# usamec/GAML

Hardware: NVIDIA B200
Metric: alignments_scored_per_s (higher is better)
Workload: dtype f64

## Files before the change

gaml_b200/csrc/engine.cu:

```cuda
#include <cuda_runtime.h>
#include <dlfcn.h>

#include <algorithm>
#include <atomic>
#include <climits>
#include <limits>
#include <cmath>
#include <cstdio>
#include <chrono>
#include <cstring>
#include <memory>
#include <memory_resource>
#include <string>
#include <unordered_map>
#include <unordered_set>
#include <vector>

#include "../../include/gaml_b200.h"
#include "kernels.h"
#include "walk_set.h"

namespace gaml {
namespace {

// ... 153 lines not shown
  bool pstar_valid = false;
  DevBuf d_qthr;
  DevBuf d_comb, d_partner12, d_partner21;
  bool comb_ok = false;
  DevBuf d_t2pack;
  bool t2pack_ok = false;
  uint32_t t2base[3] = {0, 0, 0};
  bool pairs_ok = false;
  bool lens_uniform = false;
  uint32_t uniform_ll = 0;
  int32_t class_begin[17] = {0};
  uint32_t cbase[2][5] = {{0}};
  int n_complex = 0;
  bool complex_dirty = true;
  int ins_n = 0;
  double floor_a = 0, floor_b = 0;
  DevBuf d_state_acc;
  bool total_valid = false;
  int total_two_len = 0;
  bool has_state = false;
  FlatCache flat_cache;
  int bad_bases = 0;
  bool penalty = false;
  bool sharded = false;
  bool penalty_pending = false;
  std::vector<unsigned long long> h_type1;
  DevBuf d_cov_thr, d_ev, d_ev_sorted, d_ev_temp, d_bad;
  bool pb_penalty = false;
  DevBuf d_pb_ikey, d_pb_iend, d_pb_pkey, d_pb_packed, d_pb_runmax, d_pb_temp, d_pb_count;
  std::vector<int4> h_pb_seeds, h_pb_occ;
  std::vector<uint32_t> h_pb_prefix;
  std::vector<int> h_pb_walk_len;
  std::vector<int> h_bad;
  cudaEvent_t ev0 = nullptr, ev1 = nullptr;
  ~ReadSetState() {
    for (cudaEvent_t e : {ev0, ev1})
      if (e) cudaEventDestroy(e);
  }
};

struct SetPlan {
  bool full = true;
  bool delta_only = false;
  int n_erased = 0;
  int total_len = 0;
  int64_t records = 0;
  int64_t touch_records = 0;
  int64_t records1 = 0;
  int n_cov_walks = 0, n_type1 = 0;
  uint32_t ev_cap = 0;
  size_t type1_off = 0, csbegin_off = 0, cs_off = 0, evcount_off = 0;
  int grid = 0;
  int cgrid = 0;
  size_t occ_off[2] = {0, 0};
  size_t touch_off = 0, prefix_off = 0;
  size_t pstar_off = 0;
  int n_touch = 0;
  size_t pb_seeds_off = 0, pb_occ_off = 0, pb_prefix_off = 0, pb_len_off = 0;
  uint32_t pb_cap = 0;
  size_t mtouch_off = 0, mprefix_off = 0;
  int n_mtouch = 0, n_mtouch1 = 0;
  int64_t multi_records = 0;
};

}
}
// ... 42 lines not shown
  DevBuf d_flags, d_scratch, d_csr_temp, d_logtab;
  DevBuf d_batch_blob, d_batch_acc, d_batch_out;
  DevBuf d_aln[8];
  std::vector<double> h_batch_out;
  void* h_append_pinned = nullptr;
  size_t h_append_cap = 0;
  cudaEvent_t ev_append = nullptr;
  bool append_copy_pending = false;
  double* h_out = nullptr;
  double* d_out_mapped = nullptr;
  std::vector<double> h_res;
  double* exch_host = nullptr;
  double* exch_dev = nullptr;
  int exch_rank = 0, exch_world = 1;
  bool exch_owned = false;
  DevBuf d_peer_lines, d_peer_table;
  std::vector<void*> peer_ptrs;
  std::vector<char> peer_opened;
  int peer_rank = 0, peer_world = 0;
  bool peer_on = false;
  unsigned long long* h_gather = nullptr;
  unsigned long long* d_gather_mapped = nullptr;
  void* nccl_lib = nullptr;
  void* nccl_comm = nullptr;
  int nccl_rank = 0, nccl_world = 0;
  bool nccl_on = false;
  DevBuf d_part, d_part_sum;
  unsigned long long exchange_timeout_ns = 20ull * 1000 * 1000 * 1000;
  struct GraphEntry { cudaGraph_t graph = nullptr; cudaGraphExec_t exec = nullptr; std::vector<cudaGraphNode_t> nodes; };
  std::unordered_map<uint64_t, GraphEntry> graphs;
  bool use_graphs = true;
  bool running_total = true;
  bool timing_pending = false;
  size_t h_out_cap = 0;
  unsigned long long scratch_entries = 1ull << 22;
  uint32_t ovf_cap = 1u << 20;
  uint32_t epoch = 0;
  uint32_t stamp_gen = 0;
  bool capacity_grew = false;
  bool prepared = false, launched = false;
  std::vector<SetPlan> plan;
  WalkSet wsets[2];
  int cur_set = 0;
  WalkSet& cur() { return wsets[cur_set]; }
  WalkSet& prev() { return wsets[cur_set ^ 1]; }
  std::vector<SlotUpdate> h_updates;
  std::vector<std::vector<Occ>> h_occs;
  std::vector<std::vector<TouchRange>> h_touches, h_mtouches;
  std::vector<OccBuilder> h_ob;
  std::vector<WalkView> h_refs;
  std::vector<Walk> h_walks;
  bool fast_changes = true;
  bool permute_reads = true;
  bool append_enabled = true;
  HashCounts prev_counts;
  bool have_prev = false;
  WalkDiff cur_diff;
  int prev_total_len = 0, cur_total_len = 0;
  Changes h_changes;
  alignas(16) char pool_buf[1 << 18];
  std::pmr::monotonic_buffer_resource pool{pool_buf, sizeof(pool_buf)};
  int n_updates = 0;
  size_t upd_off = 0, blob_bytes = 0;
  gaml_stats stats{};
};

// ... 1609 lines not shown
  CU(cudaGetLastError());
  return GAML_OK;
}

int nccl_all_reduce_doubles(gaml_ctx* ctx, double* buf, size_t count) {
  NcclApi* api = nccl_api(&ctx->error);
  if (!api || !ctx->nccl_comm) return fail(ctx, GAML_ERR_STATE, "no NCCL communicator: gaml_nccl_exchange_init first");
  const int rc = api->all_reduce(buf, buf, count,  8,  0, ctx->nccl_comm, ctx->stream);
  if (rc != 0) return fail(ctx, GAML_ERR_CUDA, std::string("ncclAllReduce: ") + (api->get_error_string ? api->get_error_string(rc) : "error"));
  return GAML_OK;
}

int ensure_gather_area(gaml_ctx* ctx, int world) {
  if (ctx->h_gather) return GAML_OK;
  (void)world;
  const size_t words = ((size_t)64 * GAML_EXCHANGE_MAX_SETS + 1) * kResultStride;
  CU(cudaHostAlloc(reinterpret_cast<void**>(&ctx->h_gather), words * 8, cudaHostAllocMapped));
  memset(ctx->h_gather, 0, words * 8);
  CU(cudaHostGetDevicePointer(reinterpret_cast<void**>(&ctx->d_gather_mapped), ctx->h_gather, 0));
  return GAML_OK;
}

int launch(gaml_ctx* ctx) {
  if (!ctx->prepared) return fail(ctx, GAML_ERR_STATE, "gaml_eval_launch without gaml_eval_prepare");
  cudaStream_t st = ctx->stream;
  const size_t n_sets = ctx->sets.size();
  if (ctx->timeline) {
    CU(ctx->d_timeline.reserve(kTimelineWords * 8, 0, true, st));
    CU(cudaMemsetAsync(ctx->d_timeline.p, 0, kTimelineWords * 8, st));
  }
  char* blob = ctx->blob_dev;
  int launches = 0;
  bool any_penalty = false;
  for (auto& rs : ctx->sets) any_penalty |= rs->penalty || rs->pb_penalty;
  LaunchList chain;
  const bool record = ctx->use_graphs && !ctx->profile && !any_penalty && ctx->sets.size() <= 3;
  struct RecorderGuard { ~RecorderGuard() { set_launch_recorder(nullptr); } } recorder_guard;
  if (record) set_launch_recorder(&chain);
  else if (ctx->timed) CU(cudaEventRecord(ctx->ev[0], st));
  launch_apply_slots(reinterpret_cast<const SlotUpdate*>(blob + ctx->upd_off), ctx->n_updates,
                     reinterpret_cast<const SlotUpdate*>(blob + ctx->patch_upd_off), ctx->n_patch,
                     reinterpret_cast<const int32_t*>(blob + ctx->patch_skip_off), ctx->n_skip, ctx->d_tables.as<SlotA*>(),
                     ctx->d_tables.as<SlotB*>() + ctx->stores.size(), ctx->d_tables.as<SlotA*>() + 2 * ctx->stores.size(),
                     ctx->d_tables.as<const int32_t*>() + 3 * ctx->stores.size(),
                     ctx->stores.size() <= (size_t)kInlineStores ? &ctx->h_tables : nullptr, ctx->epoch, ctx->d_flags.as<unsigned long long>(),
                     (int)flags_words(n_sets), ctx->timeline ? ctx->d_timeline.as<unsigned long long>() : nullptr, st);
  launches++;
  int64_t records = 0, reads = 0, bytes = 0;
  bool any_full = false;
  const bool profile = ctx->profile;
  bool chained = true;
  for (size_t s = 0; s < n_sets; s++) {
    ReadSetState& rs = *ctx->sets[s];
    const SetPlan& sp = ctx->plan[s];
    ScoreParams P = make_params(ctx, s);
    const int og = overflow_grid(ctx->sm_count);
    records += sp.records;
    reads += rs.n_local;
    if (rs.penalty) {
      CU(rs.d_ev.reserve((size_t)sp.ev_cap * 8, 0, false, st));
      CU(rs.d_ev_sorted.reserve((size_t)sp.ev_cap * 8, 0, false, st));
      CU(rs.d_ev_temp.reserve(std::max<size_t>(coverage_sort_temp_bytes(sp.ev_cap), 256), 0, false, st));
      CU(rs.d_bad.reserve(std::max<size_t>(sp.n_cov_walks, 1) * 4, 0, false, st));
      P.ev_keys = rs.d_ev.as<unsigned long long>();
      CU(cudaMemsetAsync(rs.d_ev.p, 0xff, (size_t)sp.ev_cap * 8, st));
      CU(cudaMemsetAsync(rs.d_bad.p, 0, std::max<size_t>(sp.n_cov_walks, 1) * 4, st));
      if (sp.n_type1) CU(cudaMemcpyAsync(rs.d_ev.p, blob + sp.type1_off, (size_t)sp.n_type1 * 8, cudaMemcpyDeviceToDevice, st));
      CU(cudaMemcpyAsync(P.ev_count, blob + sp.evcount_off, 4, cudaMemcpyDeviceToDevice, st));
      chained = false;
    }
    if (rs.cfg.kind == GAML_KIND_PAIRED) {
      if (sp.full) {
        const uint32_t n_multi = (uint32_t)sp.multi_records;
        launches += launch_paired_full(P, sp.grid, sp.cgrid, n_multi, og, ctx->sm_count, st, chained, profile, rs.ev0, rs.ev1);
        any_full = true;
        bytes += 16 * sp.records + 12 * (int64_t)rs.n_local;
      } else {
        launch_paired_delta(P, (uint32_t)sp.touch_records, sp.grid, og, ctx->sm_count, st, chained, profile, rs.ev0, rs.ev1);
        launches += sp.delta_only ? (sp.touch_records > 0 ? 2 : 1) : (sp.touch_records > 0 ? 3 : 1);
        bytes += 16 * sp.records + (sp.delta_only ? 0 : 12 * (int64_t)rs.n_local);
      }
      if (rs.penalty && rs.sharded) {
        chained = false;
      } else if (rs.penalty) {
        CU(launch_coverage(rs.d_ev.as<unsigned long long>(), rs.d_ev_sorted.as<unsigned long long>(), sp.ev_cap, rs.d_ev_temp.p,
                           rs.d_ev_temp.cap, reinterpret_cast<const int*>(blob + sp.csbegin_off),
                           reinterpret_cast<const int*>(blob + sp.cs_off), rs.cfg.step,
                           rs.cfg.insert_mean + 5 * rs.cfg.insert_std, rs.d_bad.as<int>(), ctx->sm_count, st));
        launches += 3;
        chained = false;
      } else {
        chained = !(profile && !sp.full);
      }
    } else if (rs.cfg.kind == GAML_KIND_SINGLE) {
      launch_single_full(P, sp.grid, sp.cgrid, og, st, chained, profile, rs.ev0, rs.ev1);
      chained = true;
      launches += 2 + (sp.cgrid > 0);
      bytes += 16 * sp.records + 12 * (int64_t)rs.n_local;
    } else {
      launch_pacbio_full(P, sp.grid, og, st, chained, profile, rs.ev0, rs.ev1);
      chained = true;
      launches += 2;
      if (rs.pb_penalty) {
        const size_t cap = sp.pb_cap;
        CU(rs.d_pb_ikey.reserve(cap * 2 * 8, 0, false, st));
        CU(rs.d_pb_iend.reserve(cap * 2 * 4, 0, false, st));
        CU(rs.d_pb_pkey.reserve(cap * 4 * 8, 0, false, st));
// ... 29 lines not shown
    }
  }
  if (ctx->peer_on && n_sets > 0) {
    const unsigned long long* gen = ctx->d_peer_lines.as<unsigned long long>() +
                                    (size_t)(ctx->epoch & 1u) * (size_t)ctx->peer_world * GAML_EXCHANGE_MAX_SETS * kResultStride;
    launch_exchange_gather(gen, ctx->peer_world, (int)n_sets, GAML_EXCHANGE_MAX_SETS, ctx->epoch, ctx->d_gather_mapped,
                           ctx->d_gather_mapped + (size_t)ctx->peer_world * GAML_EXCHANGE_MAX_SETS * kResultStride,
                           ctx->exchange_timeout_ns, st);
    launches++;
  }
  if (record) {
    set_launch_recorder(nullptr);
    const int rc = replay_chain(ctx, chain);
    if (rc != GAML_OK) return rc;
  }
  if (!record && ctx->timed) CU(cudaEventRecord(ctx->ev[3], st));
  if (nccl_lines(ctx) && n_sets > 0) {
    const int rc = nccl_reduce_lines(ctx, (int)n_sets);
    if (rc != GAML_OK) return rc;
    launches++;
  }
  CU(cudaGetLastError());
  ctx->stats.kernel_launches += launches;
  ctx->stats.last_records_gathered = records;
  ctx->stats.last_reads_scanned = reads;
  ctx->stats.last_algorithmic_bytes = bytes;
  ctx->stats.last_was_full = any_full ? 1 : 0;
  for (size_t s = 0; s < n_sets; s++)
    if (ctx->plan[s].delta_only) ctx->stats.delta_only_evals++;
  ctx->launched = true;
  return GAML_OK;
}

int wait_line(gaml_ctx* ctx, const volatile uint64_t* line, uint64_t want_bits, double* dst, bool own) {
  unsigned spins = 0;
  const auto t0 = std::chrono::steady_clock::now();
  for (;;) {
    uint64_t w[8];
    for (int j = 0; j < 8; j++) w[j] = line[j];
    uint64_t sum = kResultSeal;
    for (int j = 0; j < 7; j++) sum ^= w[j];
    if (w[6] == want_bits && w[7] == sum) {
      memcpy(dst, w, sizeof(w));
      return GAML_OK;
    }
    cpu_relax();
    if ((++spins & 0x3fffu) == 0) {
      const cudaError_t q = cudaStreamQuery(ctx->stream);
      if (q != cudaSuccess && q != cudaErrorNotReady) {
        ctx->error = std::string("evaluation failed on the device: ") + cudaGetErrorString(q);
        return GAML_ERR_CUDA;
      }
      const double waited = std::chrono::duration<double>(std::chrono::steady_clock::now() - t0).count();
      if (own && q == cudaSuccess && waited > 1.0) return fail(ctx, GAML_ERR_CUDA, "evaluation finished without publishing its result");
      if (!own && waited > 60.0) return fail(ctx, GAML_ERR_STATE, "a peer rank did not publish its result within 60 s");
    }
  }
}

int finish(gaml_ctx* ctx, double* partials, int32_t* total_len, double* gathered = nullptr) {
  if (!ctx->launched) return fail(ctx, GAML_ERR_STATE, "gaml_eval_finish without gaml_eval_launch");
  const size_t n_sets = ctx->sets.size();
  if (gathered && !ctx->exch_host && !ctx->peer_on && !ctx->nccl_on)
    return fail(ctx, GAML_ERR_STATE, "gaml_eval_finish_gathered needs a result exchange (gaml_set_result_exchange, gaml_peer_exchange_open "
                                     "or gaml_nccl_exchange_init)");
  const double want_d = (double)ctx->epoch;
  uint64_t want_bits;
  memcpy(&want_bits, &want_d, 8);
  const int gather_world = ctx->peer_on ? ctx->peer_world : (ctx->nccl_on ? ctx->nccl_world : ctx->exch_world);
  const bool peer_gather = gathered && ctx->peer_on;
  if (peer_gather) {
    const size_t flag_at = (size_t)ctx->peer_world * GAML_EXCHANGE_MAX_SETS * kResultStride;
    double flag[kResultStride];
    const int rc = wait_line(ctx, reinterpret_cast<const volatile uint64_t*>(ctx->h_gather + flag_at), want_bits, flag, true);
    if (rc != GAML_OK) return rc;
    std::atomic_thread_fence(std::memory_order_acquire);
// ... 5 lines not shown
      return fail(ctx, GAML_ERR_STATE, "a peer rank did not publish its result in time (ranks out of lockstep?)");
    }
  }
  const double* own_lines = peer_gather ? reinterpret_cast<const double*>(ctx->h_gather) + (size_t)ctx->peer_rank * n_sets * kResultStride
                            : (ctx->exch_host ? ctx->exch_host + exch_line(ctx, ctx->exch_rank, 0) * kResultStride : ctx->h_out);
  bool need_sync = false;
  for (size_t s = 0; s < n_sets; s++) {
    ReadSetState& rs = *ctx->sets[s];
    if ((rs.pb_penalty || rs.penalty) && rs.sharded) {
      rs.penalty_pending = true;
      need_sync = true;
      continue;
    }
    if (rs.pb_penalty) {
      rs.h_bad.assign(1, 0);
      CU(cudaMemcpyAsync(rs.h_bad.data(), rs.d_bad.p, 4, cudaMemcpyDeviceToHost, ctx->stream));
      need_sync = true;
      continue;
    }
    if (!rs.penalty) continue;
    rs.h_bad.assign(std::max(ctx->plan[s].n_cov_walks, 1), 0);
    if (ctx->plan[s].n_cov_walks)
      CU(cudaMemcpyAsync(rs.h_bad.data(), rs.d_bad.p, (size_t)ctx->plan[s].n_cov_walks * 4, cudaMemcpyDeviceToHost, ctx->stream));
    need_sync = true;
  }
  ctx->h_res.resize(std::max<size_t>(n_sets, 1) * kResultStride);
  if (need_sync) {
    CU(cudaStreamSynchronize(ctx->stream));
    memcpy(ctx->h_res.data(), own_lines, n_sets * kResultStride * sizeof(double));
  } else if (peer_gather) {
    memcpy(ctx->h_res.data(), own_lines, n_sets * kResultStride * sizeof(double));
  } else {
    const volatile uint64_t* ho = reinterpret_cast<const volatile uint64_t*>(own_lines);
    for (size_t s = 0; s < n_sets; s++) {
      const int rc = wait_line(ctx, ho + s * kResultStride, want_bits, ctx->h_res.data() + s * kResultStride, true);
      if (rc != GAML_OK) return rc;
    }
    std::atomic_thread_fence(std::memory_order_acquire);
  }
  if (gathered) {
    for (int rk = 0; rk < gather_world; rk++)
      for (size_t s = 0; s < n_sets; s++) {
        double line[kResultStride];
        if (nccl_lines(ctx)) {
          if (rk == 0) {
            const int rc = wait_line(ctx, reinterpret_cast<const volatile uint64_t*>(ctx->h_gather + s * kResultStride), want_bits, line, true);
            if (rc != GAML_OK) return rc;
            if (((uint64_t)line[5]) & 15) {
              for (auto& rsp : ctx->sets) rsp->has_state = rsp->total_valid = false;
            }
          } else {
            memset(line, 0, sizeof(line));
          }
        } else if (peer_gather) {
          memcpy(line, reinterpret_cast<const double*>(ctx->h_gather) + ((size_t)rk * n_sets + s) * kResultStride, sizeof(line));
          if (rk != ctx->peer_rank && (((uint64_t)line[5]) & 15)) return fail(ctx, GAML_ERR_CAPACITY, "a peer rank reported a capacity error");
        } else if (rk == ctx->exch_rank) {
          memcpy(line, ctx->h_res.data() + s * kResultStride, sizeof(line));
        } else {
          const volatile uint64_t* src = reinterpret_cast<const volatile uint64_t*>(ctx->exch_host + exch_line(ctx, rk, s) * kResultStride);
          const int rc = wait_line(ctx, src, want_bits, line, false);
          if (rc != GAML_OK) return rc;
          if (((uint64_t)line[5]) & 15) return fail(ctx, GAML_ERR_CAPACITY, "a peer rank reported a capacity error");
        }
        for (int k = 0; k < GAML_PARTIAL_DOUBLES; k++) gathered[((size_t)rk * n_sets + s) * GAML_PARTIAL_DOUBLES + k] = line[k];
      }
  }
  ctx->stats.last_d2h_bytes = (int64_t)(n_sets * kResultStride * sizeof(double));
  ctx->timing_pending = ctx->timed;
  if (!ctx->timed) ctx->stats.last_device_ms = ctx->stats.last_score_kernel_ms = 0;
  ctx->stats.evals++;
  ctx->prepared = ctx->launched = false;
  int tl = 0;
  uint32_t flags = 0, ovf = 0;
  int64_t scratch_placements = 0;
  bool any_paired = false;
  for (size_t s = 0; s < n_sets; s++) {
    ReadSetState& rs = *ctx->sets[s];
    const double* o = ctx->h_res.data() + s * kResultStride;
    if (partials)
      for (int k = 0; k < GAML_PARTIAL_DOUBLES; k++) partials[s * GAML_PARTIAL_DOUBLES + k] = o[k];
    const uint64_t f = (uint64_t)o[5];
    flags |= (uint32_t)(f & 15);
    ovf += (uint32_t)((f >> 4) & 0xffffff);
    scratch_placements = std::max<int64_t>(scratch_placements, (int64_t)(f >> 28));
    if (rs.pb_penalty && !rs.sharded) rs.bad_bases = rs.h_bad[0];
    if (rs.cfg.kind == GAML_KIND_PAIRED) {
      if (rs.penalty && !rs.sharded) {
        if (ctx->plan[s].full) rs.bad_bases = 0;
        for (int w = 0; w < ctx->plan[s].n_cov_walks; w++)
          rs.bad_bases += w < ctx->plan[s].n_erased ? -rs.h_bad[w] : rs.h_bad[w];
      }
      {
        const int tl1 = ctx->plan[s].total_len == 0 ? 1 : ctx->plan[s].total_len;
        rs.total_two_len = (int)(2u * (unsigned)tl1);
        rs.total_valid = true;
      }
      rs.has_state = true;
      any_paired = true;
    }
  }
  if (any_paired) {
    const WalkSet& now = ctx->cur();
    const WalkDiff& d = ctx->cur_diff;
    if (ctx->have_prev && d.valid && ctx->prev_counts.valid && !ctx->prev_counts.crowded()) {
      const WalkSet& was = ctx->prev();
      for (int i : d.old_changed) ctx->prev_counts.add(was.hash[i], -1);
      for (int i : d.new_changed) ctx->prev_counts.add(now.hash[i], +1);
    } else {
      ctx->prev_counts.rebuild(now);
    }
    ctx->prev_total_len = ctx->cur_total_len;
    ctx->cur_set ^= 1;
    ctx->have_prev = true;
    ctx->cur_diff.valid = false;
  }
  for (int kind = 0; kind < 3; kind++)
    for (size_t s = 0; s < n_sets; s++)
      if (ctx->sets[s]->cfg.kind == kind) tl = ctx->plan[s].total_len;
  if (total_len) *total_len = tl;
// ... 1435 lines not shown
}

int gaml_set_profiling(gaml_ctx* ctx, int32_t level) {
  if (check_ctx(ctx)) return GAML_ERR_ARG;
  ctx->timed = level == 1 || level == 2;
  ctx->profile = level == 2;
  ctx->timeline = level == 3;
  return GAML_OK;
}

int gaml_read_timeline(gaml_ctx* ctx, double* out_us, int32_t n) {
  if (check_ctx(ctx) || !out_us || n < kTimelineWords) return GAML_ERR_ARG;
  if (!ctx->timeline || !ctx->d_timeline.p) return fail(ctx, GAML_ERR_STATE, "gaml_set_profiling(ctx, 3) and one evaluation first");
  cudaSetDevice(ctx->device);
  CU(cudaMemcpyAsync(ctx->h_timeline, ctx->d_timeline.p, kTimelineWords * 8, cudaMemcpyDeviceToHost, ctx->stream));
  CU(cudaStreamSynchronize(ctx->stream));
  unsigned long long t0 = ~0ull;
  for (int k = 0; k < kTimelineWords; k += 2)
    if (ctx->h_timeline[k]) t0 = std::min(t0, ~ctx->h_timeline[k]);
  for (int k = 0; k < kTimelineWords; k += 2) {
    const bool ran = ctx->h_timeline[k] != 0;
    out_us[k] = ran ? (double)(~ctx->h_timeline[k] - t0) * 1e-3 : -1.0;
    out_us[k + 1] = ran ? (double)(ctx->h_timeline[k + 1] - t0) * 1e-3 : -1.0;
  }
  return GAML_OK;
}

int gaml_get_stats(gaml_ctx* ctx, gaml_stats* out) {
  if (check_ctx(ctx) || !out) return GAML_ERR_ARG;
  if (ctx->timing_pending) {
    cudaSetDevice(ctx->device);
    float ms = 0, ms2 = 0;
    if (cudaEventSynchronize(ctx->ev[3]) == cudaSuccess) cudaEventElapsedTime(&ms, ctx->ev[0], ctx->ev[3]);
    if (ctx->profile)
      for (auto& rs : ctx->sets) {
        float t = 0;
        if (cudaEventElapsedTime(&t, rs->ev0, rs->ev1) == cudaSuccess) ms2 += t;
      }
    ctx->stats.last_device_ms = ms;
    ctx->stats.last_score_kernel_ms = ms2;
    ctx->timing_pending = false;
  }
  ctx->stats.cache_appends = ctx->stats.cache_rebuilds = 0;
  for (auto& rs : ctx->sets) {
    ctx->stats.cache_appends += rs->appends;
    ctx->stats.cache_rebuilds += rs->rebuilds;
  }
  *out = ctx->stats;
  return GAML_OK;
}

}
```

gaml_b200/csrc/kernels.cu:

```cuda
#include <cub/device/device_radix_sort.cuh>
#include <cub/device/device_scan.cuh>

#include <chrono>
#include <cstdio>
#include <cstdlib>
#include <cstring>
#include <type_traits>
#include <utility>

#include "kernels.h"

namespace gaml {

namespace {

constexpr int kCapLong = 8;
constexpr int kBlock = 256;
constexpr int kOvfBlock = 128;

__device__ __forceinline__ int4 ldg4(const void* p) { return __ldg(reinterpret_cast<const int4*>(p)); }
__device__ __forceinline__ uint4 ldg_stream(const uint4* p) {
  uint4 v;
  asm volatile("ld.global.nc.L1::no_allocate.v4.u32 {%0,%1,%2,%3}, [%4];" : "=r"(v.x), "=r"(v.y), "=r"(v.z), "=r"(v.w) : "l"(p));
  return v;
// ... 72 lines not shown
  __syncthreads();
  if (threadIdx.x == 0) {
    unsigned __int128 x = 0;
#pragma unroll
    for (int j = 0; j < 8; j++) x += (unsigned __int128)sm[j] << (16 * j);
#pragma unroll
    for (int j = 0; j < 4; j++) {
      const unsigned long long limb = (unsigned long long)(unsigned)(x >> (32 * j));
      if (limb) atomicAdd(accum + j, limb);
    }
    if (sm[8]) atomicAdd(accum + 4, (unsigned long long)(long long)(int)sm[8]);
    if (sm[9]) atomicAdd(accum + 5, (unsigned long long)(long long)(int)sm[9]);
    if (sm[10]) atomicAdd(accum + 6, (unsigned long long)(long long)(int)sm[10]);
  }
}

struct PublishArgs {
  const unsigned long long* accum;
  unsigned long long* state_acc;
  double* out;
  const uint32_t* error_flag;
  const uint32_t* ovf_count;
  const unsigned long long* scratch_cursor;
  uint32_t* ticket;
  uint32_t* done;
  uint32_t epoch;
  int32_t state_add;
  long long ql;
  long long n_reads;
  unsigned long long* const* peer_bufs;
  int32_t peer_world;
  uint32_t peer_line;
  double* part_out;
};
__device__ __forceinline__ PublishArgs publish_args(const ScoreParams& P, uint32_t* ticket) {
  return PublishArgs{P.accum, P.state_acc, P.out, P.error_flag, P.ovf_count, P.scratch_cursor, ticket, P.done, P.epoch, P.state_add,
                     P.ql, (long long)P.n_reads, P.peer_bufs, P.peer_world, P.peer_line, P.part_out};
}

__device__ __noinline__ void publish_set(PublishArgs A) {
  const int lane = threadIdx.x & 31;
  unsigned long long w[8] = {0, 0, 0, 0, 0, 0, 0, 0};
  if (lane == 0) {
    __threadfence();
    unsigned long long a[7];
    for (int j = 0; j < 7; j++) a[j] = __ldcg(A.accum + j);
    unsigned __int128 x = 0;
    for (int j = 0; j < 4; j++) x += (unsigned __int128)a[j] << (32 * j);
    if (A.state_acc) {
      if (A.state_add) {
        x += ((unsigned __int128)__ldcg(A.state_acc + 1) << 64) | (unsigned __int128)__ldcg(A.state_acc);
        for (int j = 4; j < 7; j++) a[j] += __ldcg(A.state_acc + j - 2);
      }
      A.state_acc[0] = (unsigned long long)x;
      A.state_acc[1] = (unsigned long long)(x >> 64);
      for (int j = 4; j < 7; j++) A.state_acc[j - 2] = a[j];
    }
    const long long n_log = A.n_reads - (long long)a[4] - (long long)a[5] - (long long)a[6];
    const __int128 v = (__int128)x - (__int128)n_log * (__int128)A.ql;
    const unsigned __int128 xv = (unsigned __int128)v;
    const unsigned long long scratch = __ldcg(A.scratch_cursor);
    w[0] = (unsigned long long)__double_as_longlong((double)(long long)(v >> 40));
    w[1] = (unsigned long long)__double_as_longlong((double)(unsigned long long)(xv & (((unsigned __int128)1 << 40) - 1)));
    w[2] = (unsigned long long)__double_as_longlong((double)a[4]);
    w[3] = (unsigned long long)__double_as_longlong((double)a[5]);
    w[4] = (unsigned long long)__double_as_longlong((double)a[6]);
    w[5] = (unsigned long long)__double_as_longlong((double)__ldcg(A.error_flag) + 16.0 * (double)min(__ldcg(A.ovf_count), 0xffffffu) +
                                                    268435456.0 * (double)min(scratch, 0xffffffull));
    w[6] = (unsigned long long)__double_as_longlong((double)A.epoch);
    w[7] = kResultSeal;
    for (int j = 0; j < 7; j++) w[7] ^= w[j];
  }
  unsigned long long mine = 0;
#pragma unroll
  for (int j = 0; j < 8; j++) {
    const unsigned long long v = __shfl_sync(0xffffffffu, w[j], 0);
    if (lane == j) mine = v;
  }
  if (lane < 8) reinterpret_cast<unsigned long long*>(A.out)[lane] = mine;
  if (A.part_out && lane < 8) reinterpret_cast<unsigned long long*>(A.part_out)[lane] = mine;
  if (A.peer_bufs) {
    for (int p = 0; p < A.peer_world; p++) {
      unsigned long long* dst = A.peer_bufs[p] + (size_t)A.peer_line * kResultStride;
      if (lane < 8) dst[lane] = mine;
    }
    __threadfence_system();
  }
}

__global__ void __launch_bounds__(kResultStride * 32) exchange_gather_kernel(const unsigned long long* lines, int world, int n_sets, int max_sets,
                                                                              uint32_t epoch, unsigned long long* host_lines,
                                                                              unsigned long long* host_flag, unsigned long long timeout_ns) {
  pdl_release();
  __shared__ int s_fail;
  if (threadIdx.x == 0) s_fail = 0;
  __syncthreads();
  const unsigned long long want = (unsigned long long)__double_as_longlong((double)epoch);
  const unsigned long long t0 = global_ns();
  for (int i = threadIdx.x; i < world * n_sets; i += blockDim.x) {
    const int rk = i / n_sets, st = i % n_sets;
    const volatile unsigned long long* src = lines + ((size_t)rk * max_sets + st) * kResultStride;
    unsigned long long w[8];
// ... 5 lines not shown
      for (int j = 0; j < 7; j++) sum ^= w[j];
      if (w[6] == want && w[7] == sum) break;
      if (global_ns() - t0 > timeout_ns) {
        s_fail = 1;
        break;
      }
    }
    unsigned long long* dst = host_lines + (size_t)i * kResultStride;
#pragma unroll
    for (int j = 0; j < 8; j++) dst[j] = w[j];
  }
  __threadfence_system();
  __syncthreads();
  if (threadIdx.x < 8) {
    unsigned long long w[8] = {(unsigned long long)s_fail, 0, 0, 0, 0, 0, want, kResultSeal};
    for (int j = 0; j < 7; j++) w[7] ^= w[j];
    host_flag[threadIdx.x] = w[threadIdx.x];
  }
}

__global__ void reduced_publish_kernel(const double* reduced, int n_sets, uint32_t epoch, unsigned long long* host_lines) {
  const int s = blockIdx.x * blockDim.x + threadIdx.x;
  if (s >= n_sets) return;
  unsigned long long w[8];
  for (int j = 0; j < 6; j++) w[j] = (unsigned long long)__double_as_longlong(reduced[(size_t)s * kResultStride + j]);
  w[6] = (unsigned long long)__double_as_longlong((double)epoch);
  w[7] = kResultSeal;
  for (int j = 0; j < 7; j++) w[7] ^= w[j];
  __threadfence_system();
  for (int j = 0; j < 8; j++) host_lines[(size_t)s * kResultStride + j] = w[j];
}

__device__ __noinline__ void finish_blocks(PublishArgs A, bool early) {
  __shared__ bool s_last;
  __threadfence();
  __syncthreads();
  if (threadIdx.x == 0) {
    bool last = atomicAdd(A.ticket, 1u) == gridDim.x - 1;
    if (last && early) {
      __threadfence();
      last = __ldcg(A.ovf_count) == 0;
    }
    s_last = last;
  }
  __syncthreads();
  if (!s_last || threadIdx.x >= 32) return;
  publish_set(A);
  if (early && threadIdx.x == 0) *A.done = 1u;
}
__device__ __forceinline__ void finish_set(const ScoreParams& P) { finish_blocks(publish_args(P, P.ticket2), false); }
__device__ __forceinline__ void finish_set_if_complete(const ScoreParams& P) { finish_blocks(publish_args(P, P.ticket), true); }

__device__ __noinline__ double slow_log(double v) { return log(v); }

__device__ __forceinline__ double table_log(const double2* __restrict__ tab, double v) {
  const long long ix = __double_as_longlong(v);
  if ((unsigned long long)(ix - 0x0010000000000000ll) >= 0x7fe0000000000000ull) return slow_log(v);
  const long long tmp = ix - 0x3fe6000000000000ll;
  const int i = (int)((tmp >> 45) & 127);
  const long long k = tmp >> 52;
  const double z = __longlong_as_double(ix - (tmp & 0xfff0000000000000ll));
  const double2 e = tab[i];
  const double r = fma(z, e.x, -1.0);
  double p = fma(r, 1.0 / 7.0, -1.0 / 6.0);
  p = fma(r, p, 0.2);
  p = fma(r, p, -0.25);
  p = fma(r, p, 1.0 / 3.0);
  p = fma(r, p, -0.5);
  p = fma(r * r, p, r);
  return fma((double)k, 0.693147180559945309417232121458, e.y) + p;
}

__device__ __forceinline__ void acc_term(Acc& a, unsigned& floored, const double2* log_tab, double p, double pstar, long long qthr) {
  if (p < pstar) {
    floored++;
    acc_add_q(a, qthr);
    return;
  }
  const double lg = table_log(log_tab, p);
  if (fabs(lg) < kFixLimit) acc_add_q(a, __double2ll_rn(lg * kFixScale));
  else acc_count_odd(a, lg);
// ... 2334 lines not shown
  static_assert(sizeof...(KArgs) <= sizeof(PendingLaunch::arg_ptrs) / sizeof(void*), "too many kernel arguments");
  static_assert((sizeof(KArgs) + ... + 0) + 16 * sizeof...(KArgs) <= sizeof(PendingLaunch::arg_buf), "argument buffer too small");
  PendingLaunch local;
  LaunchList* rec = g_recorder;
  PendingLaunch& pl = (rec && rec->n < 16) ? rec->item[rec->n] : local;
  pl.func = reinterpret_cast<const void*>(kernel);
  pl.grid = (unsigned)grid;
  pl.block = (unsigned)block;
  pl.pdl = pdl;
  pl.n_args = 0;
  size_t off = 0;
  (pack_arg<std::remove_cv_t<std::remove_reference_t<KArgs>>>(pl, off, static_cast<std::remove_cv_t<std::remove_reference_t<KArgs>>>(args)), ...);
  if (rec && rec->n < 16) {
    rec->n++;
    return;
  }
  issue_launch(pl, st);
}

void launch_apply_slots(const SlotUpdate* upd, int n, const SlotUpdate* patch, int n_patch, const int32_t* skip, int n_skip,
                        SlotA* const* tab_a, SlotB* const* tab_b, SlotA* const* comb_base,
                        const int32_t* const* comb_map, const StoreTables* inline_tabs, uint32_t epoch, unsigned long long* flags,
                        int n_flag_words, unsigned long long* timeline, cudaStream_t st) {
  const int m = n + n_patch > n_flag_words ? n + n_patch : n_flag_words;
  if (inline_tabs)
    launch_chain(apply_slots_kernel<true>, (m + 255) / 256, 256, st, false, upd, n, patch, n_patch, skip, n_skip, tab_a, tab_b, comb_base,
                 comb_map, *inline_tabs, epoch, flags, n_flag_words, timeline);
  else
    launch_chain(apply_slots_kernel<false>, (m + 255) / 256, 256, st, false, upd, n, patch, n_patch, skip, n_skip, tab_a, tab_b, comb_base,
                 comb_map, StoreTables{}, epoch, flags, n_flag_words, timeline);
}

int launch_paired_full(const ScoreParams& P, int grid, int cgrid, uint32_t n_multi_items, int ovf_grid, int sm_count,
                       cudaStream_t st, bool chained, bool profile, cudaEvent_t e0, cudaEvent_t e1) {
  int n_launched = 0;
  (void)cgrid;
  ScoreParams Q = P;
  bool dep = chained && !profile;
  bool first = true;
  if (n_multi_items > 0 || P.n_appx > 0) {
    Q.chain_first = 1;
    Q.finish_here = 0;
    if (n_multi_items < (uint32_t)P.n_appx) n_multi_items = (uint32_t)P.n_appx;
    static const int per_sm = resident_blocks(paired_multi_kernel, kOvfBlock);
    launch_chain(paired_multi_kernel, grid_for(n_multi_items, kOvfBlock, sm_count, per_sm), kOvfBlock, st, dep, Q);
    n_launched++;
    dep = true;
    first = false;
  }
  if (profile) cudaEventRecord(e0, st);
  Q.chain_first = first || profile ? 1 : 0;
  Q.finish_here = profile ? 0 : 1;
  {
    static StreamKernel seen[16];
    static int seen_per_sm[16];
    static int n_seen = 0;
    auto blocks_per_sm = [&](StreamKernel k) {
      for (int i = 0; i < n_seen; i++)
        if (seen[i] == k) return seen_per_sm[i];
      const int v = resident_blocks(k, kBlock);
      if (n_seen < 16) { seen[n_seen] = k; seen_per_sm[n_seen++] = v; }
      return v;
    };
    const bool tab = P.pairs != nullptr && P.comb != nullptr && P.fast != nullptr;
    const StreamKernel k = stream_kernel(P.ev_keys != nullptr, P.pairs != nullptr, tab);
    if (k) {
      grid = grid_for((size_t)P.n_reads, kBlock, sm_count, blocks_per_sm(k));
      launch_chain(k, grid, kBlock, st, dep && !profile, Q);
      n_launched++;
    } else {
      ScoreParams Q1 = Q;
      Q1.finish_here = 0;
      const StreamKernel k1 = stream_kernel_tier1(), k2 = stream_kernel_rest();
      launch_chain(k1, grid_for((size_t)std::max(P.n_tier1, 1), kBlock, sm_count, blocks_per_sm(k1)), kBlock, st, dep && !profile, Q1);
      ScoreParams Q2 = Q;
      Q2.chain_first = 0;
      const int items = std::max(std::max(P.n_main, P.n_complex - P.n_main), std::max(P.n_cross / 2, P.n_appx));
      launch_chain(k2, grid_for((size_t)std::max(items, 1), kBlock, sm_count, blocks_per_sm(k2)), kBlock, st, true, Q2);
      n_launched += 2;
    }
  }
  if (profile) cudaEventRecord(e1, st);
  launch_chain(paired_overflow_kernel, ovf_grid, kOvfBlock, st, !profile, P, 1);
  return n_launched + 1;
}

void launch_paired_delta(const ScoreParams& P, uint32_t n_touch_records, int grid_total, int ovf_grid, int sm_count,
                         cudaStream_t st, bool chained, bool profile, cudaEvent_t e0, cudaEvent_t e1) {
  if (profile) cudaEventRecord(e0, st);
  bool dep = chained && !profile;
  if (n_touch_records > 0) {
    static const int per_sm = resident_blocks(paired_delta_kernel, kOvfBlock);
    launch_chain(paired_delta_kernel, grid_for(n_touch_records, kOvfBlock, sm_count, per_sm), kOvfBlock, st, dep, P);
    dep = true;
  }
  if (P.delta_only) {
    launch_chain(paired_overflow_kernel, n_touch_records > 0 ? ovf_grid : 1, kOvfBlock, st, dep, P, 2);
  } else {
    if (n_touch_records > 0) launch_chain(paired_overflow_kernel, ovf_grid, kOvfBlock, st, true, P, 0);
    launch_chain(paired_total_kernel, grid_total, kBlock, st, dep, P);
  }
  if (profile) cudaEventRecord(e1, st);
}

void launch_single_full(const ScoreParams& P, int grid, int cgrid, int ovf_grid, cudaStream_t st, bool chained, bool profile,
                        cudaEvent_t e0, cudaEvent_t e1) {
  if (profile) cudaEventRecord(e0, st);
  launch_chain(single_full_kernel, grid, kBlock, st, chained && !profile, P);
  if (cgrid > 0) launch_chain(single_complex_kernel, cgrid, kBlock, st, true, P);
  if (profile) cudaEventRecord(e1, st);
  launch_chain(single_overflow_kernel, ovf_grid, kOvfBlock, st, !profile, P);
}

void launch_pacbio_full(const ScoreParams& P, int grid, int ovf_grid, cudaStream_t st, bool chained, bool profile, cudaEvent_t e0,
                        cudaEvent_t e1) {
  if (profile) cudaEventRecord(e0, st);
  launch_chain(pacbio_full_kernel, grid, kBlock, st, chained && !profile, P);
// ... 400 lines not shown
```

gaml_b200/csrc/kernels.h:

```cpp
#pragma once
#include <cuda_runtime.h>

#include "device_types.h"

namespace gaml {

struct PendingLaunch {
  const void* func = nullptr;
  unsigned grid = 1, block = 1;
  bool pdl = false;
  int n_args = 0;
  void* arg_ptrs[16];
  alignas(16) unsigned char arg_buf[1536];
};
struct LaunchList {
  PendingLaunch item[16];
  int n = 0;
};
void set_launch_recorder(LaunchList* list);
cudaError_t issue_launch(const PendingLaunch& pl, cudaStream_t st);

enum { kGridPairedFull = 0, kGridPairedComplex, kGridPairedTotal, kGridSingleFull, kGridSingleComplex, kGridPacbioFull };
int score_grid(int which, int n_items, int sm_count);
int overflow_grid(int sm_count);

constexpr int kInlineStores = 8;
struct StoreTables {
  SlotA* a[kInlineStores];
  SlotB* b[kInlineStores];
  SlotA* cb[kInlineStores];
  const int32_t* cm[kInlineStores];
};
void launch_apply_slots(const SlotUpdate* upd, int n, const SlotUpdate* patch, int n_patch, const int32_t* skip, int n_skip,
                        SlotA* const* tab_a, SlotB* const* tab_b, SlotA* const* comb_base,
                        const int32_t* const* comb_map, const StoreTables* inline_tabs, uint32_t epoch, unsigned long long* flags,
                        int n_flag_words, unsigned long long* timeline, cudaStream_t st);
constexpr int kTimelineWords = 12;
int launch_paired_full(const ScoreParams& P, int grid, int cgrid, uint32_t n_multi_items, int ovf_grid, int sm_count,
                       cudaStream_t st, bool chained, bool profile, cudaEvent_t e0, cudaEvent_t e1);
void launch_paired_delta(const ScoreParams& P, uint32_t n_touch_records, int grid_total, int ovf_grid, int sm_count, cudaStream_t st,
                         bool chained, bool profile, cudaEvent_t e0, cudaEvent_t e1);
void launch_single_full(const ScoreParams& P, int grid, int cgrid, int ovf_grid, cudaStream_t st, bool chained, bool profile,
                        cudaEvent_t e0, cudaEvent_t e1);
void launch_pacbio_full(const ScoreParams& P, int grid, int ovf_grid, cudaStream_t st, bool chained, bool profile, cudaEvent_t e0,
                        cudaEvent_t e1);

cudaError_t build_csr(const void* arena, size_t n_records, int n_reads, bool is_long, uint32_t* rowptr, uint32_t* cursor,
                      void* rows, void* first, void* temp, size_t temp_bytes, int sm_count, cudaStream_t st, int* launches);
cudaError_t build_complex_list(const void* first1, const void* first2, int n_reads, uint32_t* flags, uint32_t* list,
                               void* temp, size_t temp_bytes, cudaStream_t st, int* launches, uint32_t* n_complex_out,
                               int32_t* class_begin);
void launch_pack_tier2(const void* cdesc, const void* rows1, const void* rows2, const int32_t* class_begin, const uint32_t cbase[2][5],
                       const uint32_t tbase[3], void* out, uint32_t* bad, cudaStream_t st);
void launch_pack_pairs(const void* first1, const void* first2, int n, const int32_t* partner12, void* out, uint32_t* bad, cudaStream_t st);
void launch_cdesc_fill(const uint32_t* list, int n_complex, const uint32_t* lens, const uint32_t* cptr1, const uint32_t* cptr2,
                       void* desc, cudaStream_t st);
cudaError_t compact_offsets(const uint32_t* list, int n_complex, const uint32_t* rowptr, uint32_t* cptr, const uint32_t* lens,
                            uint32_t* clens, void* temp, size_t temp_bytes, cudaStream_t st, int* launches);
cudaError_t compact_copy(const uint32_t* list, int n_complex, const uint32_t* rowptr, const uint32_t* cptr, const void* rows,
                         void* crows, cudaStream_t st, int* launches);
void launch_batch(const ScoreParams& P, const BatchParams& B, uint32_t n_touch_records, double* out, const uint32_t* error_flag,
                  int sm_count, cudaStream_t st);
int batch_hist_bins(int n_len);
int batch_launches(int n_len, bool touch);
void launch_build_term_table(const double* p1, const double* p2, const double* ins, int ins_n, int shift, const void* log_tab, void* out,
                             int sm_count, cudaStream_t st);
cudaError_t build_fast_pairs(const void* pairs, int n, int shift, int ins_n, uint32_t uniform_ll, void* fast, uint32_t* flags, uint32_t* list,
                             void* temp, size_t temp_bytes, cudaStream_t st, int* launches);
struct AppendGroupHost { uint32_t read, new_begin, n_new, dst; };
struct AppendMate {
  const void* arena_src; void* arena_dst; uint32_t n_rec;
  const void* groups; int n_groups; const void* new_rows; void* rows; void* first;
// ... 30 lines not shown
```

Measured before the change: 137.5 billion.

## Launch paired overflow tail kernel on demand instead of every full evaluation

When graphs are recorded and no peer/NCCL exchange is active, the paired full path now omits the overflow kernel from the chain. The main kernel publishes a 'pending' result (negative epoch) if overflow entries exist, and the host then launches the tail kernel and waits again. A per-set keep_tail flag, set from the previous overflow count, keeps the tail in the chain when overflow was seen last time. This removes an always-present launch from the common path, but adds a host round trip when overflow does occur, and the extra tail time is added to the reported timing.

```diff
diff --git a/gaml_b200/csrc/engine.cu b/gaml_b200/csrc/engine.cu
--- a/gaml_b200/csrc/engine.cu
+++ b/gaml_b200/csrc/engine.cu
@@ -209,6 +209,10 @@
   std::vector<uint32_t> h_pb_prefix;
   std::vector<int> h_pb_walk_len;
   std::vector<int> h_bad;
+  bool keep_tail = false;
+  bool tail_on_demand = false;
+  ScoreParams tail_params{};
+  int tail_grid = 0;
   cudaEvent_t ev0 = nullptr, ev1 = nullptr;
   ~ReadSetState() {
     for (cudaEvent_t e : {ev0, ev1})
@@ -317,6 +321,7 @@
   bool use_graphs = true;
   bool running_total = true;
   bool timing_pending = false;
+  bool tail_timed = false;
   size_t h_out_cap = 0;
   unsigned long long scratch_entries = 1ull << 22;
   uint32_t ovf_cap = 1u << 20;
@@ -1992,7 +1997,11 @@
   char* blob = ctx->blob_dev;
   int launches = 0;
   bool any_penalty = false;
-  for (auto& rs : ctx->sets) any_penalty |= rs->penalty || rs->pb_penalty;
+  for (auto& rs : ctx->sets) {
+    any_penalty |= rs->penalty || rs->pb_penalty;
+    rs->tail_on_demand = false;
+  }
+  ctx->tail_timed = false;
   LaunchList chain;
   const bool record = ctx->use_graphs && !ctx->profile && !any_penalty && ctx->sets.size() <= 3;
   struct RecorderGuard { ~RecorderGuard() { set_launch_recorder(nullptr); } } recorder_guard;
@@ -2032,7 +2041,13 @@
     if (rs.cfg.kind == GAML_KIND_PAIRED) {
       if (sp.full) {
         const uint32_t n_multi = (uint32_t)sp.multi_records;
-        launches += launch_paired_full(P, sp.grid, sp.cgrid, n_multi, og, ctx->sm_count, st, chained, profile, rs.ev0, rs.ev1);
+        rs.tail_on_demand = record && !ctx->peer_on && !nccl_lines(ctx) && !rs.keep_tail;
+        if (rs.tail_on_demand) {
+          rs.tail_params = P;
+          rs.tail_grid = og;
+        }
+        launches += launch_paired_full(P, sp.grid, sp.cgrid, n_multi, og, ctx->sm_count, st, chained, profile, rs.ev0, rs.ev1,
+                                       !rs.tail_on_demand);
         any_full = true;
         bytes += 16 * sp.records + 12 * (int64_t)rs.n_local;
       } else {
@@ -2128,7 +2143,8 @@
   return GAML_OK;
 }
 
-int wait_line(gaml_ctx* ctx, const volatile uint64_t* line, uint64_t want_bits, double* dst, bool own) {
+int wait_line(gaml_ctx* ctx, const volatile uint64_t* line, uint64_t want_bits, double* dst, bool own, bool* pending = nullptr,
+              uint64_t pend_bits = 0) {
   unsigned spins = 0;
   const auto t0 = std::chrono::steady_clock::now();
   for (;;) {
@@ -2136,8 +2152,10 @@
     for (int j = 0; j < 8; j++) w[j] = line[j];
     uint64_t sum = kResultSeal;
     for (int j = 0; j < 7; j++) sum ^= w[j];
-    if (w[6] == want_bits && w[7] == sum) {
+    const bool alt = pending && w[6] == pend_bits;
+    if ((w[6] == want_bits || alt) && w[7] == sum) {
       memcpy(dst, w, sizeof(w));
+      if (pending) *pending = alt;
       return GAML_OK;
     }
     cpu_relax();
@@ -2209,9 +2227,35 @@
     memcpy(ctx->h_res.data(), own_lines, n_sets * kResultStride * sizeof(double));
   } else {
     const volatile uint64_t* ho = reinterpret_cast<const volatile uint64_t*>(own_lines);
+    const double pend_d = -(double)ctx->epoch;
+    uint64_t pend_bits;
+    memcpy(&pend_bits, &pend_d, 8);
+    bool any_pending = false;
     for (size_t s = 0; s < n_sets; s++) {
-      const int rc = wait_line(ctx, ho + s * kResultStride, want_bits, ctx->h_res.data() + s * kResultStride, true);
+      ReadSetState& rs = *ctx->sets[s];
+      bool pending = false;
+      const int rc = wait_line(ctx, ho + s * kResultStride, want_bits, ctx->h_res.data() + s * kResultStride, true,
+                               rs.tail_on_demand ? &pending : nullptr, pend_bits);
       if (rc != GAML_OK) return rc;
+      if (!pending) continue;
+      if (!any_pending && ctx->timed) CU(cudaEventRecord(ctx->ev[1], ctx->stream));
+      any_pending = true;
+      launch_paired_tail(rs.tail_params, rs.tail_grid, ctx->stream);
+      CU(cudaGetLastError());
+      ctx->stats.kernel_launches++;
+    }
+    if (any_pending) {
+      if (ctx->timed) {
+        CU(cudaEventRecord(ctx->ev[2], ctx->stream));
+        ctx->tail_timed = true;
+      }
+      for (size_t s = 0; s < n_sets; s++) {
+        uint64_t flag;
+        memcpy(&flag, ctx->h_res.data() + s * kResultStride + 6, 8);
+        if (!ctx->sets[s]->tail_on_demand || flag != pend_bits) continue;
+        const int rc = wait_line(ctx, ho + s * kResultStride, want_bits, ctx->h_res.data() + s * kResultStride, true);
+        if (rc != GAML_OK) return rc;
+      }
     }
     std::atomic_thread_fence(std::memory_order_acquire);
   }
@@ -2263,6 +2307,7 @@
     scratch_placements = std::max<int64_t>(scratch_placements, (int64_t)(f >> 28));
     if (rs.pb_penalty && !rs.sharded) rs.bad_bases = rs.h_bad[0];
     if (rs.cfg.kind == GAML_KIND_PAIRED) {
+      if (ctx->plan[s].full) rs.keep_tail = ((f >> 4) & 0xffffff) != 0;
       if (rs.penalty && !rs.sharded) {
         if (ctx->plan[s].full) rs.bad_bases = 0;
         for (int w = 0; w < ctx->plan[s].n_cov_walks; w++)
@@ -3764,6 +3809,11 @@
     cudaSetDevice(ctx->device);
     float ms = 0, ms2 = 0;
     if (cudaEventSynchronize(ctx->ev[3]) == cudaSuccess) cudaEventElapsedTime(&ms, ctx->ev[0], ctx->ev[3]);
+    if (ctx->tail_timed) {
+      float t = 0;
+      if (cudaEventSynchronize(ctx->ev[2]) == cudaSuccess && cudaEventElapsedTime(&t, ctx->ev[1], ctx->ev[2]) == cudaSuccess) ms += t;
+      ctx->tail_timed = false;
+    }
     if (ctx->profile)
       for (auto& rs : ctx->sets) {
         float t = 0;
diff --git a/gaml_b200/csrc/kernels.cu b/gaml_b200/csrc/kernels.cu
--- a/gaml_b200/csrc/kernels.cu
+++ b/gaml_b200/csrc/kernels.cu
@@ -128,13 +128,14 @@
   int32_t peer_world;
   uint32_t peer_line;
   double* part_out;
+  int32_t last_in_chain;
 };
 __device__ __forceinline__ PublishArgs publish_args(const ScoreParams& P, uint32_t* ticket) {
   return PublishArgs{P.accum, P.state_acc, P.out, P.error_flag, P.ovf_count, P.scratch_cursor, ticket, P.done, P.epoch, P.state_add,
-                     P.ql, (long long)P.n_reads, P.peer_bufs, P.peer_world, P.peer_line, P.part_out};
-}
-
-__device__ __noinline__ void publish_set(PublishArgs A) {
+                     P.ql, (long long)P.n_reads, P.peer_bufs, P.peer_world, P.peer_line, P.part_out, P.finish_here == 2};
+}
+
+__device__ __noinline__ void publish_set(PublishArgs A, bool pending) {
   const int lane = threadIdx.x & 31;
   unsigned long long w[8] = {0, 0, 0, 0, 0, 0, 0, 0};
   if (lane == 0) {
@@ -143,7 +144,7 @@
     for (int j = 0; j < 7; j++) a[j] = __ldcg(A.accum + j);
     unsigned __int128 x = 0;
     for (int j = 0; j < 4; j++) x += (unsigned __int128)a[j] << (32 * j);
-    if (A.state_acc) {
+    if (A.state_acc && !pending) {
       if (A.state_add) {
         x += ((unsigned __int128)__ldcg(A.state_acc + 1) << 64) | (unsigned __int128)__ldcg(A.state_acc);
         for (int j = 4; j < 7; j++) a[j] += __ldcg(A.state_acc + j - 2);
@@ -163,7 +164,7 @@
     w[4] = (unsigned long long)__double_as_longlong((double)a[6]);
     w[5] = (unsigned long long)__double_as_longlong((double)__ldcg(A.error_flag) + 16.0 * (double)min(__ldcg(A.ovf_count), 0xffffffu) +
                                                     268435456.0 * (double)min(scratch, 0xffffffull));
-    w[6] = (unsigned long long)__double_as_longlong((double)A.epoch);
+    w[6] = (unsigned long long)__double_as_longlong(pending ? -(double)A.epoch : (double)A.epoch);
     w[7] = kResultSeal;
     for (int j = 0; j < 7; j++) w[7] ^= w[j];
   }
@@ -235,21 +236,25 @@
 }
 
 __device__ __noinline__ void finish_blocks(PublishArgs A, bool early) {
-  __shared__ bool s_last;
+  __shared__ bool s_last, s_pending;
   __threadfence();
   __syncthreads();
   if (threadIdx.x == 0) {
     bool last = atomicAdd(A.ticket, 1u) == gridDim.x - 1;
+    bool pending = false;
     if (last && early) {
       __threadfence();
-      last = __ldcg(A.ovf_count) == 0;
+      pending = __ldcg(A.ovf_count) != 0;
+      last = !pending || A.last_in_chain;
     }
     s_last = last;
+    s_pending = pending;
   }
   __syncthreads();
   if (!s_last || threadIdx.x >= 32) return;
-  publish_set(A);
-  if (early && threadIdx.x == 0) *A.done = 1u;
+  const bool pending = s_pending;
+  publish_set(A, pending);
+  if (early && !pending && threadIdx.x == 0) *A.done = 1u;
 }
 __device__ __forceinline__ void finish_set(const ScoreParams& P) { finish_blocks(publish_args(P, P.ticket2), false); }
 __device__ __forceinline__ void finish_set_if_complete(const ScoreParams& P) { finish_blocks(publish_args(P, P.ticket), true); }
@@ -2650,9 +2655,10 @@
 }
 
 int launch_paired_full(const ScoreParams& P, int grid, int cgrid, uint32_t n_multi_items, int ovf_grid, int sm_count,
-                       cudaStream_t st, bool chained, bool profile, cudaEvent_t e0, cudaEvent_t e1) {
+                       cudaStream_t st, bool chained, bool profile, cudaEvent_t e0, cudaEvent_t e1, bool tail) {
   int n_launched = 0;
   (void)cgrid;
+  tail = tail || profile;
   ScoreParams Q = P;
   bool dep = chained && !profile;
   bool first = true;
@@ -2668,7 +2674,7 @@
   }
   if (profile) cudaEventRecord(e0, st);
   Q.chain_first = first || profile ? 1 : 0;
-  Q.finish_here = profile ? 0 : 1;
+  Q.finish_here = profile ? 0 : (tail ? 1 : 2);
   {
     static StreamKernel seen[16];
     static int seen_per_sm[16];
@@ -2699,8 +2705,13 @@
     }
   }
   if (profile) cudaEventRecord(e1, st);
+  if (!tail) return n_launched;
   launch_chain(paired_overflow_kernel, ovf_grid, kOvfBlock, st, !profile, P, 1);
   return n_launched + 1;
+}
+
+void launch_paired_tail(const ScoreParams& P, int ovf_grid, cudaStream_t st) {
+  launch_chain(paired_overflow_kernel, ovf_grid, kOvfBlock, st, false, P, 1);
 }
 
 void launch_paired_delta(const ScoreParams& P, uint32_t n_touch_records, int grid_total, int ovf_grid, int sm_count,
diff --git a/gaml_b200/csrc/kernels.h b/gaml_b200/csrc/kernels.h
--- a/gaml_b200/csrc/kernels.h
+++ b/gaml_b200/csrc/kernels.h
@@ -37,7 +37,9 @@
                         int n_flag_words, unsigned long long* timeline, cudaStream_t st);
 constexpr int kTimelineWords = 12;
 int launch_paired_full(const ScoreParams& P, int grid, int cgrid, uint32_t n_multi_items, int ovf_grid, int sm_count,
-                       cudaStream_t st, bool chained, bool profile, cudaEvent_t e0, cudaEvent_t e1);
+                       cudaStream_t st, bool chained, bool profile, cudaEvent_t e0, cudaEvent_t e1,
+                       bool tail);
+void launch_paired_tail(const ScoreParams& P, int ovf_grid, cudaStream_t st);
 void launch_paired_delta(const ScoreParams& P, uint32_t n_touch_records, int grid_total, int ovf_grid, int sm_count, cudaStream_t st,
                          bool chained, bool profile, cudaEvent_t e0, cudaEvent_t e1);
 void launch_single_full(const ScoreParams& P, int grid, int cgrid, int ovf_grid, cudaStream_t st, bool chained, bool profile,
```

Measured after the change: 144.9 billion (median of 6 runs). 5.4% higher.
